# krm01/Snappy.jl

Hardware: NVIDIA B200
Metric: compress+uncompress GB/s (1 GiB synth mixed buffer; uncompressed bytes / (t_compress + t_uncompress)) (higher is better)
Workload: dtype u8

## Files before the change

### snappy.jl_b200/csrc/compress_window.cuh

```cuda
#pragma once
#include <type_traits>
#include "compress_chain.cuh"

namespace sb200 {

constexpr u32 kRingChunk = 512;
constexpr u32 kRingAhead = 64;
constexpr u32 kRingMirror = 32;
#ifndef SB200_FAR_ALL
#define SB200_FAR_ALL 1
#endif
constexpr bool kFarAll = SB200_FAR_ALL != 0;
#ifdef SB200_CPU_EMU_STATS
static unsigned long g_emu_dist[17], g_emu_dist_hit[17];
#endif
#ifdef SB200_CPU_EMU
static unsigned long g_emu_rounds = 0, g_emu_second = 0;
#endif
#ifndef SB200_M_BRANCHFREE
#define SB200_M_BRANCHFREE 1
#endif
#ifndef SB200_M_ONE_FFS
#define SB200_M_ONE_FFS 1
#endif

template <int kSmemTable, bool kLib = false, bool kSlowCont = false, bool kTwo = false>
struct Win : Chain<kSmemTable, kLib> {
    using Base = Chain<kSmemTable, kLib>;
    using Base::F;
    using Base::lane;
    using Base::lim;
    using Base::n;
    u32 Rs, rmask, lo, hi, nstage;
    bool aligned16;
    uint4 pre;
    u32 pre_at;

#ifdef SB200_CPU_EMU
    static u32 lds32(u32 a) { return *reinterpret_cast<const u32*>(smem + a); }
    template <int kOff>
    static u32 lds32o(u32 a) { return *reinterpret_cast<const u32*>(smem + a + kOff); }
    static void sts128(u32 a, uint4 v) { memcpy(smem + a, &v, 16); }
    static u32 lds8(u32 a) { return smem[a]; }
#else
    static __device__ __forceinline__ u32 lds32(u32 a) {
        u32 v;
        asm volatile("ld.shared.u32 %0, [%1];" : "=r"(v) : "r"(a) : "memory");
        return v;
    }
    template <int kOff>
    static __device__ __forceinline__ u32 lds32o(u32 a) {
        u32 v;
        asm volatile("ld.shared.u32 %0, [%1+%2];" : "=r"(v) : "r"(a), "n"(kOff) : "memory");
        return v;
    }
#endif
    __device__ __forceinline__ u32 ring32u(u32 p) const {
        const u32 a = Rs + ((p & ~3u) & rmask);
        return __funnelshift_r(lds32o<0>(a), lds32o<4>(a), p << 3);
    }
    __device__ __forceinline__ uint4 load_chunk(u32 p) const {
        uint4 v;
        if (aligned16) {
            v = __ldg(reinterpret_cast<const uint4*>(F + p));
        } else {
            v.x = ldg32u(F + p);
            v.y = ldg32u(F + p + 4);
            v.z = ldg32u(F + p + 8);
            v.w = ldg32u(F + p + 12);
        }
        return v;
    }
    __device__ __forceinline__ void stage_to(u32 upto) {
        u32 from = lo;
        if (upto > hi + rmask + 1u) {
            hi = (upto - (rmask + 1u)) & ~(kRingChunk - 1u);
            from = hi;
            pre_at = 0xffffffffu;
        }
        while (hi < upto && hi < nstage) {
            const u32 p = hi + lane * 16u;
            const uint4 v = (pre_at == hi) ? pre : load_chunk(p);
            const u32 ro = p & rmask;
#ifdef SB200_CPU_EMU
            sts128(Rs + ro, v);
            if (ro < kRingMirror) sts128(Rs + rmask + 1u + ro, v);
#else
            asm volatile("st.shared.v4.u32 [%0], {%1, %2, %3, %4};" ::"r"(Rs + ro), "r"(v.x), "r"(v.y),
                         "r"(v.z), "r"(v.w)
                         : "memory");
            if (ro < kRingMirror)
                asm volatile("st.shared.v4.u32 [%0], {%1, %2, %3, %4};" ::"r"(Rs + rmask + 1u + ro), "r"(v.x),
                             "r"(v.y), "r"(v.z), "r"(v.w)
                             : "memory");
#endif
            hi += kRingChunk;
            if (hi < nstage) {
                pre = load_chunk(hi + lane * 16u);
                pre_at = hi;
            }
        }
        lo = hi > rmask + 1u ? hi - (rmask + 1u) : 0u;
        if (lo < from) lo = from;
        __syncwarp();
    }

    __device__ __forceinline__ u32 extend(u32 ip, u32 cand, u32 M) const {
        while (ip + M < n) {
            u32 x, y;
            if (cand + M >= lo && ip + M + 32u <= hi) {
#ifdef SB200_CPU_EMU
                x = lds8(Rs + ((cand + M + lane) & rmask));
                y = lds8(Rs + ((ip + M + lane) & rmask));
#else
                asm volatile("ld.shared.u8 %0, [%1];" : "=r"(x) : "r"(Rs + ((cand + M + lane) & rmask)) : "memory");
                asm volatile("ld.shared.u8 %0, [%1];" : "=r"(y) : "r"(Rs + ((ip + M + lane) & rmask)) : "memory");
#endif
            } else {
                x = __ldg(F + cand + M + lane);
                y = __ldg(F + ip + M + lane);
            }
            const u32 nq = __ballot_sync(kFullMask, x != y);
            if (nq) {
                M += (u32)__ffs((int)nq) - 1u;
                break;
            }
            M += 32;
        }
        if (ip + M > n) M = n - ip;
        return M;
    }

    __device__ __forceinline__ void evaluate(const u32 q, const bool V, u32& H, u32& t, u32& m, u32& mp) const {
        u32 B0, B1, B2, B3;
        {
            const u32 qb = q & ~3u, sh = q << 3;
            const u32 ab = Rs + (qb & rmask);
            const u32 w0 = lds32o<0>(ab), w1 = lds32o<4>(ab), w2 = lds32o<8>(ab), w3 = lds32o<12>(ab),
                      w4 = lds32o<16>(ab);
            B0 = __funnelshift_r(w0, w1, sh);
            B1 = __funnelshift_r(w1, w2, sh);
            B2 = __funnelshift_r(w2, w3, sh);
            B3 = __funnelshift_r(w3, w4, sh);
        }
        H = this->hash(B0);
        t = V ? this->tget(H) : lo;
        mp = __match_any_sync(kFullMask, V ? H : (0x80000000u | lane));
        const u32 nearp = (t >= lo) ? 1u : 0u;
        const uintptr_t ga = reinterpret_cast<uintptr_t>(F + t);
        const u32* g = reinterpret_cast<const u32*>(ga & ~(uintptr_t)3);
        const u32 tb = t & ~3u, tsh = (nearp ? t : (u32)ga) << 3;
        u32 c0, c1, c2 = 0, c3 = 0, c4 = 0;
        const u32 far_all = kFarAll ? 1u : 0u;
#ifdef SB200_CPU_EMU
        if (nearp) {
            const u32 ra = Rs + (tb & rmask);
            c0 = lds32o<0>(ra); c1 = lds32o<4>(ra); c2 = lds32o<8>(ra); c3 = lds32o<12>(ra); c4 = lds32o<16>(ra);
        } else {
            c0 = g[0]; c1 = g[1];
            if (far_all) { c2 = g[2]; c3 = g[3]; c4 = g[4]; }
        }
#else
        asm volatile(
            "{\n"
            ".reg .pred p;\n"
            "setp.ne.u32 p, %5, 0;\n"
            "@p ld.shared.u32 %0, [%6];\n"
            "@p ld.shared.u32 %1, [%6+4];\n"
            "@p ld.shared.u32 %2, [%6+8];\n"
            "@p ld.shared.u32 %3, [%6+12];\n"
            "@p ld.shared.u32 %4, [%6+16];\n"
            "@!p ld.global.nc.u32 %0, [%7];\n"
            "@!p ld.global.nc.u32 %1, [%7+4];\n"
            "setp.ne.and.u32 p, %8, 0, !p;\n"
            "@p ld.global.nc.u32 %2, [%7+8];\n"
            "@p ld.global.nc.u32 %3, [%7+12];\n"
            "@p ld.global.nc.u32 %4, [%7+16];\n"
            "}\n"
            : "=r"(c0), "=r"(c1), "+r"(c2), "+r"(c3), "+r"(c4)
            : "r"(nearp), "r"(Rs + (tb & rmask)), "l"(g), "r"(far_all)
            : "memory");
#endif
        u32 C0 = __funnelshift_r(c0, c1, tsh);
        const bool more = V && !nearp && !far_all && C0 == B0;
        if (__any_sync(kFullMask, more)) {
            if (more) {
                c2 = __ldg(g + 2);
                c3 = __ldg(g + 3);
                c4 = __ldg(g + 4);
            }
        }
        m = 0;
        {
            const u32 x0 = C0 ^ B0, x1 = __funnelshift_r(c1, c2, tsh) ^ B1,
                      x2 = __funnelshift_r(c2, c3, tsh) ^ B2, x3 = __funnelshift_r(c3, c4, tsh) ^ B3;
#if SB200_M_ONE_FFS
            const u32 w = x0 ? x0 : (x1 ? x1 : (x2 ? x2 : x3));
            const u32 base = x0 ? 0u : (x1 ? 4u : (x2 ? 8u : 12u));
            m = w ? base + (((u32)__ffs((int)w) - 1u) >> 3) : 16u;
#elif SB200_M_BRANCHFREE
            const u32 m0 = x0 ? ((u32)__ffs((int)x0) - 1u) >> 3 : 4u, m1 = x1 ? ((u32)__ffs((int)x1) - 1u) >> 3 : 4u,
                      m2 = x2 ? ((u32)__ffs((int)x2) - 1u) >> 3 : 4u, m3 = x3 ? ((u32)__ffs((int)x3) - 1u) >> 3 : 4u;
            const bool f0 = m0 == 4u, f1 = f0 && m1 == 4u, f2 = f1 && m2 == 4u;
            m = m0 + (f0 ? m1 : 0u) + (f1 ? m2 : 0u) + (f2 ? m3 : 0u);
#else
            if (x0) m = ((u32)__ffs((int)x0) - 1u) >> 3;
            else if (x1) m = 4u + (((u32)__ffs((int)x1) - 1u) >> 3);
            else if (x2) m = 8u + (((u32)__ffs((int)x2) - 1u) >> 3);
            else if (x3) m = 12u + (((u32)__ffs((int)x3) - 1u) >> 3);
            else m = 16u;
#endif
            if (!V) m = 0;
        }
#ifdef SB200_CPU_EMU_STATS
        if (V) {
            const u32 dist = q - t;
            u32 b = 0;
            while ((1u << (b + 1)) <= dist && b < 16) b++;
            g_emu_dist[b]++;
            if (m >= 4u) g_emu_dist_hit[b]++;
        }
#endif
    }

    enum : u32 { K_COPY = 0, K_SLOW = 1, K_FIN = 2, K_NEXTSCAN = 3, K_NEXTARR = 4, K_LEAVE = 5 };

    __device__ __forceinline__ void run_window() {
        asm volatile("" : "+r"(this->n), "+r"(this->Ts), "+r"(this->shift), "+r"(Rs), "+r"(rmask));
        this->op = 0;
        this->nrec = 0;
        this->r_lit = this->r_cpy = 0;
        lim = (int)n - Base::kLimMargin;
        u32 lit_from = 0;
        if (n >= kInputMargin) {
            bool arrival = false;
            u32 a = 1, scan_s = 1;
            for (;;) {
                if (!arrival && a - scan_s >= 32u) {
                    u32 ip = 0, cand = 0;
                    int res = 0;
                    for (u32 base = 32; res == 0; base += 32)
                        res = this->scan_round(scan_s + g_probe_offsets[base + lane],
                                               scan_s + g_probe_offsets[base + lane + 1], true, ip, cand);
                    if (res == 2) break;
                    const u32 M = extend(ip, cand, 4);
                    this->keep(lit_from, ip, cand, M);
                    a = ip + M;
                    lit_from = a;
                    if ((int)a >= lim) break;
                    arrival = true;
                    continue;
                }
                if (a + kRingAhead + (kTwo ? 32u : 0u) > hi) stage_to(a + kRingAhead + (kTwo ? 32u : 0u));
                if (arrival) {
                    if (lane == 0) this->tput(this->hash(ring32u(a - 1u)), a - 1u);
                    __syncwarp();
                }
#ifdef SB200_CPU_EMU
                if (lane == 0) g_emu_rounds++;
#endif
                u32 q = a + lane;
                bool V = (int)q < lim;
                u32 H, t, m, mp;
                evaluate(q, V, H, t, m, mp);
                u32 H1 = 0, t1 = 0, m1 = 0, mp1 = 0;
                bool V1 = false;
                const bool have_hi = kTwo && (int)(a + 32u) < lim;
                if (have_hi) {
                    V1 = (int)(q + 32u) < lim;
                    evaluate(q + 32u, V1, H1, t1, m1, mp1);
                }
                u32 changed = 0, entry = 0;
                u32 d, insacc, cur;
                for (u32 half = 0;; half++) {
                const u32 vmask = __ballot_sync(kFullMask, V);
                const u32 hitmask = __ballot_sync(kFullMask, m >= 4u);
                const u32 dupmask = __ballot_sync(kFullMask, (mp & ((1u << lane) - 1u)) != 0u) | changed;
                const u32 tm = (t << 16) | (m << 8);
                const u32 stop_all = ~vmask | dupmask | hitmask;
                u32 desc, ins;
                {
                    const u32 lbit = 1u << lane;
                    const u32 rest = (lane < 31u) ? (stop_all >> (lane + 1u)) : 0u;
                    const u32 es = lane + (u32)__ffs((int)rest);
                    const u32 ebit = 1u << (es & 31u);
                    const bool hit = (hitmask & lbit) != 0u, none = rest == 0u;
                    const bool ev_invalid = (vmask & ebit) == 0u, ev_dup = (dupmask & ebit) != 0u;
                    const bool untrusted = (lane != 0u || half != 0u) && (dupmask & lbit) != 0u;
                    const u32 above = (lane < 31u) ? (~0u << (lane + 1u)) : 0u;
                    const u32 kind_scan = none ? (u32)K_LEAVE
                                               : (ev_invalid ? (u32)K_FIN : (ev_dup ? (u32)K_NEXTSCAN : (u32)K_COPY));
                    const u32 ins_scan = none ? above : (((ebit - 1u) & above) | ((ev_invalid || ev_dup) ? 0u : ebit));
                    u32 kind = hit ? (u32)K_COPY : kind_scan;
                    u32 e = hit ? lane : (none ? 0u : es);
                    ins = lbit | (lbit >> 1) | (hit ? 0u : ins_scan);
                    kind = untrusted ? (u32)K_NEXTARR : kind;
                    e = untrusted ? lane : e;
                    ins = untrusted ? 0u : ins;
                    const u32 r = __shfl_sync(kFullMask, tm, e);
                    if (kind == K_COPY && ((r >> 8) & 31u) == 16u) kind = K_SLOW;
                    desc = kind | (e << 3) | ((hitmask & lbit) ? 0u : (1u << 13)) | (r & 0xffff1f00u);
                }
                cur = entry;
                if (arrival) {
                    d = __shfl_sync(kFullMask, desc, entry);
                    insacc = __shfl_sync(kFullMask, ins, entry);
                } else {
                    const u32 klim = 32u - (a - scan_s);
                    const u32 limmask = klim < 32u ? ~((1u << klim) - 1u) : 0u;
                    const u32 rest = stop_all | limmask;
                    u32 kind, e = 0;
                    if (!rest) {
                        kind = K_LEAVE;
                        insacc = ~0u;
                    } else {
                        e = (u32)__ffs((int)rest) - 1u;
                        const u32 ebit = 1u << e;
                        insacc = ebit - 1u;
                        if (!(vmask & ebit)) kind = K_FIN;
                        else if ((dupmask | limmask) & ebit) kind = K_NEXTSCAN;
                        else {
                            kind = K_COPY;
                            insacc |= ebit;
                        }
                    }
                    const u32 r = __shfl_sync(kFullMask, tm, e);
                    if (kind == K_COPY && ((r >> 8) & 31u) == 16u) kind = K_SLOW;
                    d = kind | (e << 3) | (r & 0xffff1f00u);
                }
                for (;;) {
                    if (d & (1u << 13)) scan_s = a + cur + 1u;
                    if (kSlowCont && (d & 7u) == K_SLOW) {
                        const u32 e = (d >> 3) & 31u, ip = a + e, cand = d >> 16;
                        const u32 M = extend(ip, cand, 16);
                        this->keep(lit_from, ip, cand, M);
                        lit_from = ip + M;
                        if ((int)lit_from >= lim) {
                            d = K_FIN;
                            break;
                        }
                        if (e + M >= 32u) {
                            d = K_NEXTARR | (1u << 14);
                            break;
                        }
                        cur = e + M;
                        d = __shfl_sync(kFullMask, desc, cur);
                        insacc |= __shfl_sync(kFullMask, ins, cur);
                        continue;
                    }
                    if ((d & 7u) != K_COPY) break;
                    const u32 e = (d >> 3) & 31u, me = (d >> 8) & 31u;
                    this->keep(lit_from, a + e, d >> 16, me);
                    cur = e + me;
                    lit_from = a + cur;
                    if ((int)lit_from >= lim) {
                        d = K_FIN;
                        break;
                    }
                    if (cur >= 32u) {
                        d = K_NEXTARR | (1u << 14);
                        break;
                    }
                    d = __shfl_sync(kFullMask, desc, cur);
                    insacc |= __shfl_sync(kFullMask, ins, cur);
                }
                const u32 ins_all = insacc;
                if (((ins_all >> lane) & 1u) && (mp & ins_all & ~((2u << lane) - 1u)) == 0u) this->tput(H, q);
                __syncwarp();
                if (kTwo && half == 0u && have_hi) {
                    const u32 k0 = d & 7u;
                    const bool leave = k0 == K_LEAVE && a + 32u - scan_s < 32u;
                    const bool landed = k0 == K_NEXTARR && (d & (1u << 14)) && lit_from - (a + 32u) < 32u;
                    if (leave || landed) {
#ifdef SB200_CPU_EMU
                        if (lane == 0) g_emu_second++;
#endif
                        entry = landed ? lit_from - (a + 32u) : 0u;
                        arrival = landed;
                        if (landed && entry == 0u && lane == 31u) this->tput(H, q);
                        a += 32u;
                        __syncwarp();
                        const u32 tnow = V1 ? this->tget(H1) : t1;
                        changed = __ballot_sync(kFullMask, V1 && tnow != t1);
                        q += 32u;
                        V = V1;
                        H = H1;
                        t = t1;
                        m = m1;
                        mp = mp1;
                        continue;
                    }
                }
                break;
                }
                const u32 kind = d & 7u, ev = (d >> 3) & 31u;
                if (kind == K_SLOW) {
                    const u32 ip = a + ev, cand = d >> 16;
                    const u32 M = extend(ip, cand, 16);
                    this->keep(lit_from, ip, cand, M);
                    a = ip + M;
                    lit_from = a;
                    if ((int)a >= lim) break;
                    arrival = true;
                    continue;
                }
                if (kind == K_FIN) break;
                if (kind == K_LEAVE) {
                    arrival = false;
                    a += 32u;
                } else if (kind == K_NEXTSCAN) {
                    arrival = false;
                    a += ev;
                } else {
                    arrival = true;
                    a = (d & (1u << 14)) ? lit_from : a + ev;
                }
            }
        }
        this->finish(lit_from);
    }
};

struct WindowArgs {
    const u8* g_in;
    u64 shard_len;
    u32 nfrag, shift;
    const u8* tail_copy;
    u8* scratch;
    u32* frag_sizes;
    u32* counter;
    u16* gtables;
    u32 reserve;
    const ShardDesc* descs;
    u32 ndesc;
    const u32* ready;
    u32* done;
    u32 done_div;
    u32 lib_rules;
    const u32* order;
    u64* trace;
};

template <int kSmemTable, bool kLib>
struct Pipe;
template <int kSmemTable, bool kLib, bool kSlowCont, bool kTwo = false, bool kPipe = false>
__device__ __forceinline__ void window_warp_loop(const WindowArgs& A, u16* T, u32 ring, u32 ring_bytes, u32 tab,
                                                 u32 reserve, bool dyn_smem = false) {
    const bool in_smem = kSmemTable == 2 ? dyn_smem : kSmemTable == 1;
    const u32 lane = lane_id();
    const u32 nfrag = A.nfrag;
    for (;;) {
        if (reserve && *reinterpret_cast<volatile u32*>(A.counter) + reserve >= nfrag) break;
        u32 frag = 0;
        if (lane == 0) frag = atomicAdd(A.counter, 1u);
        frag = __shfl_sync(kFullMask, frag, 0);
        if (frag >= nfrag) break;
        if (A.order) frag = A.order[frag];
        u64 t_begin = 0;
#ifndef SB200_CPU_EMU
        if (A.trace) asm volatile("mov.u64 %0, %%globaltimer;" : "=l"(t_begin));
#endif
        if (A.ready) {
            if (lane == 0) {
                const u32 need = frag + 2u < nfrag ? frag + 2u : nfrag;
                while (*reinterpret_cast<const volatile u32*>(A.ready) < need) __nanosleep(500);
            }
            __syncwarp();
        }
        const u8* sbase = A.g_in;
        const u8* stail = A.tail_copy;
        u64 slen = A.shard_len;
        u32 local = frag, lastf = nfrag - 1, fshift = A.shift;
        if (A.descs) {
            u32 k = 0;
            while (k + 1 < A.ndesc && A.descs[k + 1].frag_begin <= frag) k++;
            sbase = A.descs[k].ptr;
            stail = A.descs[k].tail;
            slen = A.descs[k].len;
            local = frag - A.descs[k].frag_begin;
            lastf = A.descs[k].nfrag - 1;
            fshift = A.descs[k].shift;
        }
        const u64 start = (u64)local * kBlockSize;
        const u32 n = (u32)((slen - start < kBlockSize) ? (slen - start) : kBlockSize);
        u32 entries = 1u << (32 - fshift);
        if (kLib) {
            entries = 256;
            while (entries < tab && entries < n) entries <<= 1;
            fshift = A.lib_rules == 2u ? 17u : (u32)__clz((int)entries) + 1u;
        }
        uint4* t4 = reinterpret_cast<uint4*>(T);
        for (u32 i = lane; i < entries / 8; i += 32) t4[i] = make_uint4(0, 0, 0, 0);
        __syncwarp();
        typename std::conditional<kPipe, Pipe<kSmemTable, kLib>, Win<kSmemTable, kLib, kSlowCont, kTwo>>::type ch;
        ch.hmask = entries - 1u;
        ch.F = (local == lastf) ? stail : sbase + start;
        ch.T = T;
        ch.Ts = in_smem ? smem_u32(T) : 0u;
        ch.dyn_smem = dyn_smem;
        ch.out = A.scratch + (u64)frag * kSlotStride;
        ch.n = n;
        ch.shift = fshift;
        ch.lane = lane;
        ch.spec = 0;
        ch.make_policy();
        ch.Rs = ring;
        ch.rmask = ring_bytes - 1u;
        ch.lo = ch.hi = 0;
        ch.pre_at = 0xffffffffu;
        ch.nstage = (n + kRingChunk - 1u) & ~(kRingChunk - 1u);
        ch.aligned16 = (reinterpret_cast<uintptr_t>(ch.F) & 15u) == 0;
        if constexpr (kPipe) ch.run_pipe();
        else ch.run_window();
        if (lane == 0) A.frag_sizes[frag] = ch.op;
        if (A.trace && lane == 0) {
            u64 t_end = 0;
            u32 smid = 0;
#ifndef SB200_CPU_EMU
            asm volatile("mov.u64 %0, %%globaltimer;" : "=l"(t_end));
            asm volatile("mov.u32 %0, %%smid;" : "=r"(smid));
#endif
            A.trace[2 * (u64)frag] = (t_begin & ~(u64)1) | (in_smem ? 1u : 0u);
            A.trace[2 * (u64)frag + 1] = (t_end & ~(u64)0xff) | (smid & 0xffu);
        }
        if (A.done) {
            __threadfence();
            __syncwarp();
            if (lane == 0) atomicAdd(A.done + frag / A.done_div, 1u);
        }
        __syncwarp();
    }
}

template <bool kSmemTable, bool kLib = false, bool kSlowCont = false, bool kPipe = false>
__global__ void __launch_bounds__(kSmemTable ? 224 : 640, 1)
k_compress_window(const WindowArgs A, u32 ring_bytes) {
    extern __shared__ __align__(128) u8 smem[];
    const u32 warp = threadIdx.x >> 5;
    const u32 nwarp = blockDim.x >> 5;
    const u32 gwarp = blockIdx.x * nwarp + warp;
    const u32 tab = kLib ? (A.lib_rules == 2u ? 2u * kMaxTableEntries : kMaxTableEntries) : kMaxTableEntries;
    u16* T = kSmemTable ? reinterpret_cast<u16*>(smem) + (size_t)warp * tab : A.gtables + (size_t)gwarp * tab;
    const u32 ring = smem_u32(smem) + (kSmemTable ? nwarp * tab * 2u : 0u) + warp * (ring_bytes + kRingMirror);
    window_warp_loop<kSmemTable, kLib, kSlowCont, false, kPipe>(A, T, ring, ring_bytes, tab, kSmemTable ? 0u : A.reserve);
}

template <bool kLib = false, bool kTwoA = false, bool kTwoB = false, int kPipe = 0, bool kUni = false>
__global__ void __launch_bounds__(640, 1)
k_compress_window_mixed(const WindowArgs A, u32 wa, u32 wb, u32 ring_a, u32 ring_b, u32 smem_first) {
    extern __shared__ __align__(128) u8 smem[];
    const u32 warp = threadIdx.x >> 5;
    const u32 tab = kLib ? (A.lib_rules == 2u ? 2u * kMaxTableEntries : kMaxTableEntries) : kMaxTableEntries;
    const u32 rings = smem_u32(smem) + wa * tab * 2u;
    const bool is_smem = smem_first ? warp < wa : warp >= wb;
    if (kUni) {
        const u32 w = is_smem ? (smem_first ? warp : warp - wb) : (smem_first ? warp - wa : warp);
        u16* T = is_smem ? reinterpret_cast<u16*>(smem) + (size_t)w * tab : A.gtables + ((size_t)blockIdx.x * wb + w) * tab;
        const u32 ring = is_smem ? rings + w * (ring_a + kRingMirror)
                                 : rings + wa * (ring_a + kRingMirror) + w * (ring_b + kRingMirror);
        window_warp_loop<2, kLib, false, false, kPipe != 0>(A, T, ring, is_smem ? ring_a : ring_b, tab,
                                                            is_smem ? 0u : A.reserve, is_smem);
        return;
    }
    if (is_smem) {
        const u32 w = smem_first ? warp : warp - wb;
        u16* T = reinterpret_cast<u16*>(smem) + (size_t)w * tab;
        window_warp_loop<true, kLib, false, kTwoA, (kPipe & 1) != 0>(A, T, rings + w * (ring_a + kRingMirror), ring_a, tab, 0u);
    } else {
        const u32 w = smem_first ? warp - wa : warp;
        u16* T = A.gtables + ((size_t)blockIdx.x * wb + w) * tab;
        window_warp_loop<false, kLib, false, kTwoB, (kPipe & 2) != 0>(A, T, rings + wa * (ring_a + kRingMirror) + w * (ring_b + kRingMirror),
                                                    ring_b, tab, A.reserve);
    }
}

template <bool kLib = false>
__global__ void __launch_bounds__(512, 1)
k_compress_pages_window(const u8* __restrict__ g_in, const u64* __restrict__ in_off, const u32* __restrict__ in_size,
                        u32 count, u8* __restrict__ g_out, const u64* __restrict__ out_off, u32* __restrict__ out_size,
                        u32 ring_bytes, u32 table_cap, u32* __restrict__ counter, u32 lib_rules = 0) {
    extern __shared__ __align__(128) u8 smem[];
    const u32 warp = threadIdx.x >> 5;
    const u32 nwarp = blockDim.x >> 5;
    const u32 lane = lane_id();
    u16* T = reinterpret_cast<u16*>(smem) + (size_t)warp * table_cap;
    u8* R = smem + (size_t)nwarp * table_cap * 2u + (size_t)warp * (ring_bytes + kRingMirror);
    for (;;) {
        u32 pg = 0;
        if (lane == 0) pg = atomicAdd(counter, 1u);
        pg = __shfl_sync(kFullMask, pg, 0);
        if (pg >= count) break;
        const u8* pin = g_in + in_off[pg];
        const u32 n = in_size[pg];
        u8* pout = g_out + out_off[pg];
        u32 hdr = 0;
        {
            u32 v = n;
            while (v >= 0x80) {
                if (lane == 0) pout[hdr] = (u8)(v | 0x80);
                v >>= 7;
                hdr++;
            }
            if (lane == 0) pout[hdr] = (u8)v;
            hdr++;
        }
        u32 entries = 256;
        while (entries < table_cap && entries < n) entries <<= 1;
        u32 fshift = (u32)__clz((int)entries) + 1u;
        if (kLib && lib_rules == 2u) fshift = 17u;
        uint4* t4 = reinterpret_cast<uint4*>(T);
        for (u32 i = lane; i < entries / 8; i += 32) t4[i] = make_uint4(0, 0, 0, 0);
        const bool al = (reinterpret_cast<uintptr_t>(pin) & 15u) == 0;
        for (u32 i = lane * 16u; i < ring_bytes; i += 512u) {
            uint4 v = make_uint4(0, 0, 0, 0);
            if (i + 16u <= n && al) {
                v = __ldg(reinterpret_cast<const uint4*>(pin + i));
            } else if (i < n) {
                u32 w[4] = {0, 0, 0, 0};
                for (u32 k = 0; k < 16u && i + k < n; k++) w[k >> 2] |= (u32)__ldg(pin + i + k) << (8u * (k & 3u));
                v = make_uint4(w[0], w[1], w[2], w[3]);
            }
            *reinterpret_cast<uint4*>(R + i) = v;
            if (i < kRingMirror) *reinterpret_cast<uint4*>(R + ring_bytes + i) = v;
        }
        __syncwarp();
        Win<true, kLib> ch;
        ch.hmask = entries - 1u;
        ch.F = pin;
        ch.T = T;
        ch.Ts = smem_u32(T);
        ch.out = pout + hdr;
        ch.n = n;
        ch.shift = fshift;
        ch.lane = lane;
        ch.spec = 0;
        ch.make_policy();
        ch.Rs = smem_u32(R);
        ch.rmask = ring_bytes - 1u;
        ch.lo = 0;
        ch.hi = 0x7fffff00u;
        ch.pre_at = 0xffffffffu;
        ch.nstage = 0;
        ch.aligned16 = false;
        ch.run_window();
        if (lane == 0) out_size[pg] = hdr + ch.op;
        __syncwarp();
    }
}

}
```

Measured before the change: 61.56.

## Resolve duplicate-hash lanes in-window instead of rescanning

Adds resolve kinds (K_RSCAN/K_RARR) so that, when a lane's hash collides with an earlier lane in the same 32-byte window, the warp finds the in-window candidate from the match-position mask and computes the match length from the shared-memory ring with one ballot. It then continues the copy/scan decision chain in place, avoiding a fallback to another scan round or arrival pass. The scan-decision logic is factored into scan_from, which can start from any lane offset. It also adds a ring8 helper and CPU-emulation statistics counters. The cost is extra shuffles and ring reads on the resolve path, plus more branchy control flow; it only applies when neither kSlowCont nor kTwo is set.

```diff
diff --git a/snappy.jl_b200/csrc/compress_window.cuh b/snappy.jl_b200/csrc/compress_window.cuh
--- a/snappy.jl_b200/csrc/compress_window.cuh
+++ b/snappy.jl_b200/csrc/compress_window.cuh
@@ -16,6 +16,13 @@
 #endif
 #ifdef SB200_CPU_EMU
 static unsigned long g_emu_rounds = 0, g_emu_second = 0;
+enum { EMU_RES_ARR, EMU_RES_SCAN, EMU_RES_ARR_COPY, EMU_RES_ARR_SLOW, EMU_RES_ARR_MISS, EMU_RES_SCAN_HIT,
+       EMU_RES_SCAN_MISS, EMU_RES_IN_WINDOW, EMU_RES_LANE31, EMU_RES_PROBE_LIMIT, EMU_RES_NEAR_LIM, EMU_RES_BEYOND,
+       EMU_RES_FORMS };
+static const char* const g_emu_res_name[EMU_RES_FORMS] = {
+    "arrival", "scan", "arrival-copy", "arrival-slow", "arrival-miss", "scan-hit", "scan-miss", "in-window-candidate",
+    "lane31", "probe-limit", "near-lim", "copy-beyond-window"};
+static unsigned long g_emu_res[EMU_RES_FORMS];
 #endif
 #ifndef SB200_M_BRANCHFREE
 #define SB200_M_BRANCHFREE 1
@@ -55,6 +62,15 @@
         return v;
     }
 #endif
+    __device__ __forceinline__ u32 ring8(u32 p) const {
+#ifdef SB200_CPU_EMU
+        return lds8(Rs + (p & rmask));
+#else
+        u32 v;
+        asm volatile("ld.shared.u8 %0, [%1];" : "=r"(v) : "r"(Rs + (p & rmask)) : "memory");
+        return v;
+#endif
+    }
     __device__ __forceinline__ u32 ring32u(u32 p) const {
         const u32 a = Rs + ((p & ~3u) & rmask);
         return __funnelshift_r(lds32o<0>(a), lds32o<4>(a), p << 3);
@@ -109,13 +125,8 @@
         while (ip + M < n) {
             u32 x, y;
             if (cand + M >= lo && ip + M + 32u <= hi) {
-#ifdef SB200_CPU_EMU
-                x = lds8(Rs + ((cand + M + lane) & rmask));
-                y = lds8(Rs + ((ip + M + lane) & rmask));
-#else
-                asm volatile("ld.shared.u8 %0, [%1];" : "=r"(x) : "r"(Rs + ((cand + M + lane) & rmask)) : "memory");
-                asm volatile("ld.shared.u8 %0, [%1];" : "=r"(y) : "r"(Rs + ((ip + M + lane) & rmask)) : "memory");
-#endif
+                x = ring8(cand + M + lane);
+                y = ring8(ip + M + lane);
             } else {
                 x = __ldg(F + cand + M + lane);
                 y = __ldg(F + ip + M + lane);
@@ -223,7 +234,36 @@
 #endif
     }
 
-    enum : u32 { K_COPY = 0, K_SLOW = 1, K_FIN = 2, K_NEXTSCAN = 3, K_NEXTARR = 4, K_LEAVE = 5 };
+    enum : u32 { K_COPY = 0, K_SLOW = 1, K_FIN = 2, K_NEXTSCAN = 3, K_NEXTARR = 4, K_LEAVE = 5, K_RSCAN = 6, K_RARR = 7 };
+    static constexpr bool kResolve = !kSlowCont && !kTwo;
+    static constexpr u32 kScanU = kResolve ? (u32)K_RSCAN : (u32)K_NEXTSCAN, kArrU = kResolve ? (u32)K_RARR : (u32)K_NEXTARR;
+
+    __device__ __forceinline__ u32 scan_from(u32 s, u32 a, u32 scan_s, u32 stop_all, u32 vmask, u32 dupmask, u32 tm,
+                                             u32& insacc) const {
+        const u32 klim = scan_s + 32u - a;
+        const u32 limmask = klim < 32u ? ~0u << klim : 0u;
+        const u32 from = s < 32u ? ~0u << s : 0u;
+        const u32 rest = (stop_all | limmask) & from;
+        u32 kind, e = 0;
+        if (!rest) {
+            kind = K_LEAVE;
+            insacc |= from;
+        } else {
+            e = (u32)__ffs((int)rest) - 1u;
+            const u32 ebit = 1u << e;
+            insacc |= (ebit - 1u) & from;
+            if (!(vmask & ebit)) kind = K_FIN;
+            else if (limmask & ebit) kind = K_NEXTSCAN;
+            else if (dupmask & ebit) kind = kScanU;
+            else {
+                kind = K_COPY;
+                insacc |= ebit;
+            }
+        }
+        const u32 r = __shfl_sync(kFullMask, tm, e);
+        if (kind == K_COPY && ((r >> 8) & 31u) == 16u) kind = K_SLOW;
+        return kind | (e << 3) | (r & 0xffff1f00u);
+    }
 
     __device__ __forceinline__ void run_window() {
         asm volatile("" : "+r"(this->n), "+r"(this->Ts), "+r"(this->shift), "+r"(Rs), "+r"(rmask));
@@ -289,12 +329,12 @@
                     const bool untrusted = (lane != 0u || half != 0u) && (dupmask & lbit) != 0u;
                     const u32 above = (lane < 31u) ? (~0u << (lane + 1u)) : 0u;
                     const u32 kind_scan = none ? (u32)K_LEAVE
-                                               : (ev_invalid ? (u32)K_FIN : (ev_dup ? (u32)K_NEXTSCAN : (u32)K_COPY));
+                                               : (ev_invalid ? (u32)K_FIN : (ev_dup ? kScanU : (u32)K_COPY));
                     const u32 ins_scan = none ? above : (((ebit - 1u) & above) | ((ev_invalid || ev_dup) ? 0u : ebit));
                     u32 kind = hit ? (u32)K_COPY : kind_scan;
                     u32 e = hit ? lane : (none ? 0u : es);
                     ins = lbit | (lbit >> 1) | (hit ? 0u : ins_scan);
-                    kind = untrusted ? (u32)K_NEXTARR : kind;
+                    kind = untrusted ? kArrU : kind;
                     e = untrusted ? lane : e;
                     ins = untrusted ? 0u : ins;
                     const u32 r = __shfl_sync(kFullMask, tm, e);
@@ -306,28 +346,12 @@
                     d = __shfl_sync(kFullMask, desc, entry);
                     insacc = __shfl_sync(kFullMask, ins, entry);
                 } else {
-                    const u32 klim = 32u - (a - scan_s);
-                    const u32 limmask = klim < 32u ? ~((1u << klim) - 1u) : 0u;
-                    const u32 rest = stop_all | limmask;
-                    u32 kind, e = 0;
-                    if (!rest) {
-                        kind = K_LEAVE;
-                        insacc = ~0u;
-                    } else {
-                        e = (u32)__ffs((int)rest) - 1u;
-                        const u32 ebit = 1u << e;
-                        insacc = ebit - 1u;
-                        if (!(vmask & ebit)) kind = K_FIN;
-                        else if ((dupmask | limmask) & ebit) kind = K_NEXTSCAN;
-                        else {
-                            kind = K_COPY;
-                            insacc |= ebit;
-                        }
-                    }
-                    const u32 r = __shfl_sync(kFullMask, tm, e);
-                    if (kind == K_COPY && ((r >> 8) & 31u) == 16u) kind = K_SLOW;
-                    d = kind | (e << 3) | (r & 0xffff1f00u);
-                }
+                    insacc = 0;
+                    d = scan_from(0u, a, scan_s, stop_all, vmask, dupmask, tm, insacc);
+                }
+#ifdef SB200_CPU_EMU
+                bool emu_res_copy = false;
+#endif
                 for (;;) {
                     if (d & (1u << 13)) scan_s = a + cur + 1u;
                     if (kSlowCont && (d & 7u) == K_SLOW) {
@@ -348,11 +372,49 @@
                         insacc |= __shfl_sync(kFullMask, ins, cur);
                         continue;
                     }
-                    if ((d & 7u) != K_COPY) break;
+                    if ((d & 7u) != K_COPY) {
+                        if (!kResolve || (d & 7u) < K_RSCAN) break;
+                        const u32 u = (d >> 3) & 31u, ubit = 1u << u;
+                        const bool arr = (d & 7u) == K_RARR;
+                        const u32 pre = arr ? ubit >> 1 : 0u;
+                        const u32 jm = __shfl_sync(kFullMask, mp, u) & (insacc | pre) & (ubit - 1u);
+                        u32 tmu = d & 0xffff1f00u;
+                        if (jm) {
+                            const u32 cand = a + 31u - (u32)__clz((int)jm);
+                            const u32 ne = __ballot_sync(kFullMask, ring8(a + u + lane) != ring8(cand + lane)) | 0xffff0000u;
+                            tmu = (cand << 16) | (((u32)__ffs((int)ne) - 1u) << 8);
+                        }
+                        insacc |= ubit | pre;
+                        const u32 mu = (tmu >> 8) & 31u;
+#ifdef SB200_CPU_EMU
+                        if (lane == 0) {
+                            const u32 klim = scan_s + 32u - a;
+                            g_emu_res[arr ? EMU_RES_ARR : EMU_RES_SCAN]++;
+                            g_emu_res[arr ? (mu == 16u ? EMU_RES_ARR_SLOW : (mu >= 4u ? EMU_RES_ARR_COPY : EMU_RES_ARR_MISS))
+                                          : (mu >= 4u ? EMU_RES_SCAN_HIT : EMU_RES_SCAN_MISS)]++;
+                            if (jm) g_emu_res[EMU_RES_IN_WINDOW]++;
+                            if (u == 31u) g_emu_res[EMU_RES_LANE31]++;
+                            if (!arr && klim < 32u) g_emu_res[EMU_RES_PROBE_LIMIT]++;
+                            if (vmask != ~0u) g_emu_res[EMU_RES_NEAR_LIM]++;
+                        }
+                        emu_res_copy = mu >= 4u;
+#endif
+                        if (mu >= 4u) {
+                            d = (mu == 16u ? (u32)K_SLOW : (u32)K_COPY) | (u << 3) | tmu;
+                        } else {
+                            if (arr) scan_s = a + u + 1u;
+                            d = scan_from(u + 1u, a, scan_s, stop_all, vmask, dupmask, tm, insacc);
+                        }
+                        continue;
+                    }
                     const u32 e = (d >> 3) & 31u, me = (d >> 8) & 31u;
                     this->keep(lit_from, a + e, d >> 16, me);
                     cur = e + me;
                     lit_from = a + cur;
+#ifdef SB200_CPU_EMU
+                    if (lane == 0 && emu_res_copy && cur >= 32u) g_emu_res[EMU_RES_BEYOND]++;
+                    emu_res_copy = false;
+#endif
                     if ((int)lit_from >= lim) {
                         d = K_FIN;
                         break;
```

Result: slower. 60.45, median of 6 (-1.8%).
